# aleflabo/PREGO

Measured on AMD Instinct MI355X. Metric: frames/sec (per-frame action logits) on Assembly101-O TSN features, higher is better.
Workload: dtype fp16; 1 GPU; BASELINE configs[1]: Assembly101-O-test-split-shaped eval set, MiniROAD eval path (rgb+flow fp32 [T,2048] each -> per-frame probs[86] + argmax); clips_per_gpu=182, frames_per_gpu=2306143, min_T=3342, max_T=33981, flow=non-zero (full K=4096 layer1 GEMM), parallelism=clip-sharded dp1, no collective: every rank its own eval-set-sized clip list, weights=random init, seed 20

## Files before the change

prego_amd/csrc/ff_pass.hip:

```cpp
#include "common.h"
#include "kernels.h"
#include "gemm_tile.h"
#include "pass_handshake.h"

#define FF_TIMEOUT_TICKS 200000000ull

__device__ __forceinline__ bool ffp_wait_ge(const unsigned* p, unsigned need, unsigned* abort_word, unsigned code) {
  if (__hip_atomic_load(p, __ATOMIC_RELAXED, __HIP_MEMORY_SCOPE_AGENT) >= need) return true;
  const unsigned long long t0 = __builtin_amdgcn_s_memrealtime();
  unsigned spins = 0;
  for (;;) {
    __builtin_amdgcn_s_sleep(8);
    if (__hip_atomic_load(p, __ATOMIC_RELAXED, __HIP_MEMORY_SCOPE_AGENT) >= need) return true;
    if ((++spins & 31u) == 0u) {
      if (__hip_atomic_load(abort_word, __ATOMIC_RELAXED, __HIP_MEMORY_SCOPE_AGENT)) return false;
      if (__builtin_amdgcn_s_memrealtime() - t0 > FF_TIMEOUT_TICKS) {
        __hip_atomic_store(abort_word, code, __ATOMIC_RELAXED, __HIP_MEMORY_SCOPE_AGENT);
        return false;
      }
    }
  }
}

template <typename OT, bool SC1OUT>
// ... 23 lines not shown
#pragma unroll
  for (int y = 0; y < 2; ++y)
#pragma unroll
    for (int j = 0; j < 2; ++j) bv[y][j] = *(const float4*)(bias + y * 128 + wc * 32 + fq * 8 + j * 4);
  const __amdgpu_buffer_rsrc_t rs_c = __builtin_amdgcn_make_buffer_rsrc((void*)C, 0, rows * ldc * 2, 0x00020000);
#pragma unroll
  for (int x = 0; x < 2; ++x)
#pragma unroll
    for (int y = 0; y < 2; ++y) {
      const int n = y * 128 + wc * 32 + fq * 8;
#pragma unroll
      for (int i = 0; i < 4; ++i) {
        const int m = x * 128 + grp * 64 + i * 16 + fr;
        const f32x4 v0 = acc[x][y][i][0], v1 = acc[x][y][i][1];
        u32x4 pk;
        pk[0] = op16<OT>::pack2_sat(v0[0] + bv[y][0].x, v0[1] + bv[y][0].y); pk[1] = op16<OT>::pack2_sat(v0[2] + bv[y][0].z, v0[3] + bv[y][0].w);
        pk[2] = op16<OT>::pack2_sat(v1[0] + bv[y][1].x, v1[1] + bv[y][1].y); pk[3] = op16<OT>::pack2_sat(v1[2] + bv[y][1].z, v1[3] + bv[y][1].w);
        if constexpr (SC1OUT) __builtin_amdgcn_raw_buffer_store_b128(pk, rs_c, (m * ldc + n) * 2, 0, AUX_SC1);
        else __builtin_amdgcn_raw_buffer_store_b128(pk, rs_c, (m * ldc + n) * 2, 0, 0);
      }
    }
}

template <typename OT, bool IN16>
__device__ __forceinline__ void ffp_pack_rows(const FfPassArgs& a, int my_rows, int wave, int lane, const char* srgb, const char* sflow,
                                              bf16_t* __restrict__ Xs) {
  constexpr int ES = IN16 ? 2 : 4, NV = IN16 ? 1 : 2;
  constexpr int PR = 2;
  const int din = a.kx;
  const int cr_rgb = (a.d_rgb + 2047) >> 11, cpr = cr_rgb + ((a.d_flow + 2047) >> 11);
  const int n_rounds = my_rows > 0 ? ((my_rows + PR - 1) / PR) * cpr : 0;
  auto readlane_ptr = [](const char* p, int l) -> const char* {
    const unsigned long long v = (unsigned long long)p;
    const unsigned lo = (unsigned)__builtin_amdgcn_readlane((int)(unsigned)v, l), hi = (unsigned)__builtin_amdgcn_readlane((int)(unsigned)(v >> 32), l);
    return (const char*)(((unsigned long long)hi << 32) | lo);
  };
  int voff_in = lane * 8 * ES, voff_in2 = voff_in + 1024 * ES, voff_out = lane * 16;
  asm volatile("" : "+v"(voff_in), "+v"(voff_in2), "+v"(voff_out));
  auto issue = [&](u32x4 (&v)[PR][4][NV], int k) {
    const int rp = k / cpr, cj = k - rp * cpr;
    const bool fl = cj >= cr_rgb;
    const int cwin = (fl ? cj - cr_rgb : cj) << 11, seg_len = fl ? a.d_flow : a.d_rgb;
#pragma unroll
    for (int e = 0; e < PR; ++e) {
      const int r = rp * PR + e, rr = r < my_rows ? r : 0;
      const char* s0 = readlane_ptr(srgb, rr);
      const char* s1 = readlane_ptr(sflow, rr);
      const char* src = fl ? s1 : s0;
      const __amdgpu_buffer_rsrc_t rs = __builtin_amdgcn_make_buffer_rsrc((void*)(src + (size_t)cwin * ES), 0,
                                                                          (r < my_rows && src != nullptr) ? (seg_len - cwin) * ES : 0, 0x00020000);
#pragma unroll
      for (int b = 0; b < 4; ++b)
#pragma unroll
        for (int w = 0; w < NV; ++w)
          v[e][b][w] = __builtin_amdgcn_raw_buffer_load_b128(rs, (b < 2 ? voff_in : voff_in2) + ((b & 1) * 512 * ES + 16 * w), 0, AUX_NT);
    }
  };
  auto drain = [&](const u32x4 (&v)[PR][4][NV], int k) {
    const int rp = k / cpr, cj = k - rp * cpr;
    const bool fl = cj >= cr_rgb;
    const int cwin = (fl ? cj - cr_rgb : cj) << 11, seg_len = fl ? a.d_flow : a.d_rgb, seg_base = fl ? a.d_rgb : 0;
#pragma unroll
    for (int e = 0; e < PR; ++e) {
      const int r = rp * PR + e;
      bf16_t* dst = Xs + (size_t)(wave * 32 + (r < my_rows ? r : 0)) * din + seg_base + cwin;
      const __amdgpu_buffer_rsrc_t rs = __builtin_amdgcn_make_buffer_rsrc((void*)dst, 0, r < my_rows ? (seg_len - cwin) * 2 : 0, 0x00020000);
#pragma unroll
      for (int b = 0; b < 4; ++b) {
        u32x4 o = v[e][b][0];
        if constexpr (!IN16) {
          const u32x4 x = v[e][b][0], y = v[e][b][NV - 1];
          o[0] = op16<OT>::pack2_sat(__uint_as_float(x[0]), __uint_as_float(x[1])); o[1] = op16<OT>::pack2_sat(__uint_as_float(x[2]), __uint_as_float(x[3]));
          o[2] = op16<OT>::pack2_sat(__uint_as_float(y[0]), __uint_as_float(y[1])); o[3] = op16<OT>::pack2_sat(__uint_as_float(y[2]), __uint_as_float(y[3]));
        }
        __builtin_amdgcn_raw_buffer_store_b128(o, rs, voff_out + b * 1024, 0, 0);
      }
    }
  };
  u32x4 va[PR][4][NV], vb[PR][4][NV];
  if (n_rounds == 0) return;
  issue(va, 0);
  int k = 0;
#define PACK_FENCE() __builtin_amdgcn_sched_barrier(0)
  for (; k + 2 < n_rounds; k += 2) {
    issue(vb, k + 1); PACK_FENCE();
    drain(va, k); PACK_FENCE();
    issue(va, k + 2); PACK_FENCE();
    drain(vb, k + 1); PACK_FENCE();
  }
  if (k + 1 < n_rounds) {
    issue(vb, k + 1); PACK_FENCE();
    drain(va, k); PACK_FENCE();
    drain(vb, k + 1);
  } else {
    drain(va, k);
  }
#undef PACK_FENCE
}

template <typename OT>
__device__ __forceinline__ void ffp_pack(const FfPassArgs& a, int row0, int nrows, bf16_t* __restrict__ Xs) {
  int tid_ = threadIdx.x;
  asm volatile("" : "+v"(tid_));
  const int lane = tid_ & 63, wave = __builtin_amdgcn_readfirstlane(tid_ >> 6);
  const int rl = wave * 32 + (lane & 31);
  int clip = 0, t = 0;
  if (rl < nrows) {
    const int row = row0 + rl;
    int lo = a.plan.blk_step[row >> 5];
    while (lo + 1 < a.plan.s_max && a.plan.rowoff[lo + 1] <= row) ++lo;
    const int slot = row - a.plan.rowoff[lo];
    int k = a.plan.seg_off[slot];
    const int kend = a.plan.seg_off[slot + 1];
    while (k + 1 < kend && a.plan.seg_start[k + 1] <= lo) ++k;
    clip = a.plan.seg_clip[k];
    t = lo - a.plan.seg_start[k];
    if (a.rowmap != nullptr && lane < 32) ((int2*)a.rowmap)[row] = make_int2(clip, t);
  }
  const char* srgb = nullptr; const char* sflow = nullptr;
  const int es = a.in16 ? 2 : 4;
  if (rl < nrows) {
    const float* rgb = a.rgb_ptrs ? a.rgb_ptrs[clip] : nullptr;
    const float* flow = a.flow_ptrs ? a.flow_ptrs[clip] : nullptr;
    if (rgb) srgb = (const char*)rgb + (size_t)t * a.d_rgb * es;
    if (flow) sflow = (const char*)flow + (size_t)t * a.d_flow * es;
  }
  const int my_rows = nrows - wave * 32 < 32 ? nrows - wave * 32 : 32;
  if (a.in16) ffp_pack_rows<OT, true>(a, my_rows, wave, lane, srgb, sflow, Xs);
  else ffp_pack_rows<OT, false>(a, my_rows, wave, lane, srgb, sflow, Xs);
}

constexpr int FLN_MAX_E = 2048;

template <typename OT, int NV, int NR>
__device__ __forceinline__ void ffp_ln(const FfPassArgs& a, int nrows, const bf16_t* __restrict__ Ys, bf16_t* __restrict__ Es, const float* gb) {
  int tid_ = threadIdx.x;
  asm volatile("" : "+v"(tid_));
  const int lane = tid_ & 63, wave = __builtin_amdgcn_readfirstlane(tid_ >> 6);
  const int E = NV * 512;
  const float fE = (float)a.E;
  if (wave >= nrows) return;
  auto request = [&](u32x4 (&dst)[NR][NV], int rb) {
#pragma unroll
    for (int e = 0; e < NR; ++e) {
      int r = rb + 8 * e;
      if (r >= nrows) r = wave;
      const bf16_t* y = Ys + (size_t)r * E;
#pragma unroll
      for (int i = 0; i < NV; ++i) dst[e][i] = *(const u32x4*)(y + (i * 64 + lane) * 8);
    }
// ... 186 lines not shown
    default: ffp_ln_generic<OT, 8, 2>(a, nrows, Ys, Es); break;
  }
}

template <typename OT>
__global__ __launch_bounds__(512, 2) void ff_pass_kernel(FfPassArgs a) {
  extern __shared__ __attribute__((aligned(16))) char smem[];
  __shared__ int s_job[2];
  const int tid = threadIdx.x;
  const int xcc = __builtin_amdgcn_readfirstlane(__builtin_amdgcn_s_getreg((3 << 11) | 20) & 7);
  if (xcc < a.xcd_lo) return;
  if (tid == 0) {
    const unsigned nth = __hip_atomic_fetch_add(a.hs.ff_here + xcc, 1u, __ATOMIC_RELAXED, __HIP_MEMORY_SCOPE_AGENT);
    s_job[1] = hs_wait(a.hs, a.hs.ticks_all) == PREGO_HS_GO ? 1 : 0;
    if (a.max_wg > 0 && (int)nth >= a.max_wg) s_job[1] = 0;
  }
  __syncthreads();
  if (!__builtin_amdgcn_readfirstlane(s_job[1])) return;
  __shared__ __attribute__((aligned(16))) float s_gb[2 * FLN_MAX_E];
  if (a.E <= FLN_MAX_E)
    for (int c = tid; c < a.E; c += 512) { s_gb[c] = a.ln_g[c]; s_gb[FLN_MAX_E + c] = a.ln_b[c]; }
  const int q = xcc - a.xcd_lo, nf = 8 - a.xcd_lo;
  const int n_q = a.n_units > q ? (a.n_units - q + nf - 1) / nf : 0;
  const int sg = a.sg, tpr = sg * (2 + a.nt1 + a.nt2);
  const int n_rounds = (n_q + sg - 1) / sg + a.lag3;
  __shared__ unsigned long long s_stat[11];
  const bool stats = a.stats != nullptr && tid == 0;
  if (stats) {
    for (int e = 0; e < 8; ++e) s_stat[e] = 0;
    s_stat[9] = __builtin_amdgcn_s_memrealtime(); s_stat[8] = s_stat[9]; s_stat[10] = __builtin_amdgcn_s_memtime();
  }
#define FSTAT(i) do { if (stats) { const unsigned long long n_ = __builtin_amdgcn_s_memrealtime(); s_stat[i] += n_ - s_stat[8]; s_stat[8] = n_; } } while (0)
  for (;;) {
    __syncthreads();
    if (tid == 0) s_job[0] = (int)__hip_atomic_fetch_add(a.tick + q, 1u, __ATOMIC_RELAXED, __HIP_MEMORY_SCOPE_AGENT);
    __syncthreads();
    const int k = __builtin_amdgcn_readfirstlane(s_job[0]);
    const int round = k / tpr, j = k - round * tpr;
    FSTAT(5);
    if (round >= n_rounds) break;
    int type, i, nb = 0;
    if (j < sg) { type = 0; i = round * sg + j; }
    else if (j < sg + sg * a.nt1) { const int jj = j - sg; type = 1; nb = jj / sg; i = (round - a.lag1) * sg + (jj - nb * sg); }
    else if (j < 2 * sg + sg * a.nt1) { type = 2; i = (round - a.lag2) * sg + (j - sg - sg * a.nt1); }
    else { const int jj = j - 2 * sg - sg * a.nt1; type = 3; nb = jj / sg; i = (round - a.lag3) * sg + (jj - nb * sg); }
    if (i < 0 || i >= n_q) continue;
    const int u = q + i * nf;
    if (tid == 0) {
      bool ok = true;
      const int up = u - a.ring_units;
      if (type == 0) {
        if (up >= 0) ok = ffp_wait_ge(a.l1_cnt + up, (unsigned)a.nt1, a.abort_word, 0x100u);
      } else if (type == 1) {
        ok = ffp_wait_ge(a.pack_done + u, 1u, a.abort_word, 0x101u);
        if (ok && up >= 0) ok = ffp_wait_ge(a.ln_done + up, 1u, a.abort_word, 0x102u);
      } else if (type == 2) {
        ok = ffp_wait_ge(a.l1_cnt + u, (unsigned)a.nt1, a.abort_word, 0x103u);
        if (ok && up >= 0) ok = ffp_wait_ge(a.wih_cnt + up, (unsigned)a.nt2, a.abort_word, 0x104u);
      } else {
        ok = ffp_wait_ge(a.ln_done + u, 1u, a.abort_word, 0x105u);
        const int ug = u - a.gi_ring_units;
        if (ok && ug >= 0) ok = ffp_wait_ge(a.rec_cnt + (ug >> a.chunk_unit_shift), (unsigned)a.rec_expect, a.abort_word, 0x106u);
      }
      s_job[1] = ok ? 1 : 0;
    }
    __syncthreads();
    if (!__builtin_amdgcn_readfirstlane(s_job[1])) break;
    FSTAT(4);
    asm volatile("buffer_inv sc0" ::: "memory");
    const int row0 = u * 256;
    const int nrows = a.total_rows - row0 < 256 ? a.total_rows - row0 : 256;
    const size_t slot = (size_t)(u % a.ring_units) * 256;
    if (type == 0) {
      if (!(a.dbg & 1)) ffp_pack<OT>(a, row0, nrows, a.X + slot * a.kx);
    } else if (type == 1) {
      if (!(a.dbg & 4))
      ffp_tile<OT, false>(smem, a.X + slot * a.kx, a.kx, nrows, a.w1 + (size_t)nb * 256 * a.ld_w1, a.ld_w1, a.b1 + nb * 256,
                          a.Y + slot * a.E + nb * 256, a.E, a.kx);
    } else if (type == 2) {
      if (a.dbg & 2) { }
      else ffp_ln_any<OT>(a, nrows, a.Y + slot * a.E, a.Eb + slot * a.E, s_gb);
    } else {
      const size_t gslot = (size_t)(u & (a.gi_ring_units - 1)) * 256;
      if (!(a.dbg & 8))
      ffp_tile<OT, true>(smem, a.Eb + slot * a.E, a.E, nrows, a.w_ih + (size_t)nb * 256 * a.E, a.E, a.bias2 + nb * 256,
                         a.GI + gslot * a.n3 + nb * 256, a.n3, a.E);
    }
    asm volatile("s_waitcnt vmcnt(0)" ::: "memory");
    __syncthreads();
    FSTAT(type);
    if (tid == 0) {
      if (type == 0) __hip_atomic_store(a.pack_done + u, 1u, __ATOMIC_RELAXED, __HIP_MEMORY_SCOPE_AGENT);
      else if (type == 1) __hip_atomic_fetch_add(a.l1_cnt + u, 1u, __ATOMIC_RELAXED, __HIP_MEMORY_SCOPE_AGENT);
      else if (type == 2) __hip_atomic_store(a.ln_done + u, 1u, __ATOMIC_RELAXED, __HIP_MEMORY_SCOPE_AGENT);
      else {
        const unsigned old = __hip_atomic_fetch_add(a.wih_cnt + u, 1u, __ATOMIC_RELAXED, __HIP_MEMORY_SCOPE_AGENT);
        if (old + 1u == (unsigned)a.nt2)
          __hip_atomic_fetch_add(a.gi_cnt + (u >> a.chunk_unit_shift), 1u, __ATOMIC_RELAXED, __HIP_MEMORY_SCOPE_AGENT);
      }
    }
  }
  if (stats) {
    s_stat[7] = __builtin_amdgcn_s_memrealtime() - s_stat[9];
    s_stat[6] = __builtin_amdgcn_s_memtime() - s_stat[10];
    for (int e = 0; e < 8; ++e) atomicAdd(a.stats + e, s_stat[e]);
  }
#undef FSTAT
}

int launch_ff_pass(const FfPassArgs& a, hipStream_t s) {
  if (a.E % 512 || a.E > 4096 || a.kx % kPpBK || a.kx < 2 * kPpBK || a.n3 % 256 || a.xcd_lo < 1 || a.xcd_lo > 7) return -1;
  if (a.sg < 1 || a.ring_units % (8 - a.xcd_lo) || (a.gi_ring_units & (a.gi_ring_units - 1)) || a.nt1 != a.E / 256 || a.nt2 != a.n3 / 256) return -1;
  static DeviceOnce once;
  once.run([&] {
    (void)hipFuncSetAttribute((const void*)ff_pass_kernel<bf16_t>, hipFuncAttributeMaxDynamicSharedMemorySize, 2 * kPpBuf);
    (void)hipFuncSetAttribute((const void*)ff_pass_kernel<f16_t>, hipFuncAttributeMaxDynamicSharedMemorySize, 2 * kPpBuf);
  });
  if (a.f16) ff_pass_kernel<f16_t><<<256, 512, 2 * kPpBuf, s>>>(a);
  else ff_pass_kernel<bf16_t><<<256, 512, 2 * kPpBuf, s>>>(a);
  return 0;
}
```

prego_amd/csrc/head_softmax.hip:

```cpp
#include "common.h"
#include "kernels.h"
#include <cstdlib>

#define HM 4
template <typename WT, int NTC>
__global__ __launch_bounds__(256) void head_softmax_kernel(
    const WT* __restrict__ Hrelu,
    const WT* __restrict__ Wc,
    const float* __restrict__ bc,
    SlotPlan plan, int row0, int nrows, int HID, int C, int apply_softmax,
    float* const* __restrict__ out_ptrs,
    int* const* __restrict__ argmax_ptrs) {
  constexpr bool BF = (sizeof(WT) == 2);
  const int lane = threadIdx.x & 63, wave = threadIdx.x >> 6;
  const int l15 = lane & 15, l4 = lane >> 4;
  const int rbase = (blockIdx.x * 4 + wave) * 16 * HM;
  if (rbase >= nrows) return;
  int arow[HM];
#pragma unroll
  for (int m = 0; m < HM; ++m) { arow[m] = rbase + m * 16 + l15; if (arow[m] > nrows - 1) arow[m] = nrows - 1; }

  __shared__ unsigned long long s_out[4][64], s_arg[4][64];
  {
    typedef const __attribute__((address_space(4))) int* cint_p;
// ... 93 lines not shown
      for (int o = 1; o < 16; o <<= 1) s += __shfl_xor(s, o, 64);
      const float inv = 1.0f / s;
#pragma unroll
      for (int j = 0; j < NTC; ++j) v[j] *= inv;
    }
    const int rr = m * 16 + l4 * 4 + e;
    if (rbase + rr < nrows) {
      float* op = (float*)s_out[wave][rr];
      if (op) {
#pragma unroll
        for (int j = 0; j < NTC; ++j) {
          const int c = j * 16 + l15;
          if (c < C) op[c] = v[j];
        }
      }
      if (l15 == 0) {
        int* aptr = (int*)s_arg[wave][rr];
        if (aptr) *aptr = mi;
      }
    }
  }
}

template <int NTC, typename OT = bf16_t>
__global__ __launch_bounds__(256, 1) void head_softmax_v2_kernel(
    const bf16_t* __restrict__ Hrelu, const bf16_t* __restrict__ Wc, const float* __restrict__ bc, SlotPlan plan, int row0,
    int nrows, int C, int apply_softmax, float* const* __restrict__ out_ptrs, int* const* __restrict__ argmax_ptrs,
    const int2* __restrict__ rowmap ) {
  constexpr int HID = 1024, KS = 8;
  extern __shared__ __attribute__((aligned(16))) char smem[];
  f32x4* part = (f32x4*)smem;
  constexpr int PSTRIDE = 4 * 2 * NTC * 64;
  const int lane = threadIdx.x & 63, q = __builtin_amdgcn_readfirstlane(threadIdx.x >> 6);
  const int l15 = lane & 15, g = lane >> 4;
  bf16x8 wc[NTC][KS];
#pragma unroll
  for (int j = 0; j < NTC; ++j)
#pragma unroll
    for (int ks = 0; ks < KS; ++ks) wc[j][ks] = *(const bf16x8*)(Wc + (size_t)(j * 16 + l15) * HID + q * 256 + ks * 32 + 8 * g);
  float bias[NTC][4];
#pragma unroll
  for (int j = 0; j < NTC; ++j)
#pragma unroll
    for (int e = 0; e < 4; ++e) bias[j][e] = bc[j * 16 + 4 * g + e];

  const int nblk = (nrows + 31) / 32;
  const int* __restrict__ p_rowoff = plan.rowoff; const int* __restrict__ p_seg_off = plan.seg_off;
  const int* __restrict__ p_seg_clip = plan.seg_clip; const int* __restrict__ p_seg_start = plan.seg_start;
  const int* __restrict__ p_blk = plan.blk_step;
  const int s_max = plan.s_max;
  bf16x8 cur[2][KS], nxt[2][KS];
#define HEAD_LOAD(DST, BLK)                                                                                             \
  do {                                                                                                                  \
    _Pragma("unroll") for (int t = 0; t < 2; ++t) {                                                                     \
      int r_ = (BLK) * 32 + t * 16 + l15; if (r_ > nrows - 1) r_ = nrows - 1;                                           \
      _Pragma("unroll") for (int ks = 0; ks < KS; ++ks) {                                                               \
        const u32x4 v_ = __builtin_nontemporal_load((const u32x4*)(Hrelu + (size_t)r_ * HID + q * 256 + ks * 32 + 8 * g)); \
        DST[t][ks] = __builtin_bit_cast(bf16x8, v_);                                                                    \
      }                                                                                                                 \
    }                                                                                                                   \
  } while (0)
  const int rq = (q & 1) * 16 + l15;
  auto map_row = [&](int b) { int r = b * 32 + rq; return r < nrows ? r : nrows - 1; };
  int blk = blockIdx.x;
  int2 ct = make_int2(0, 0), ctn = make_int2(0, 0);
  if (blk < nblk) {
    if (rowmap != nullptr) ct = rowmap[map_row(blk)];
    HEAD_LOAD(cur, blk);
  }
  int parity = 0;
  for (; blk < nblk; blk += gridDim.x) {
    const int bn = blk + gridDim.x;
    const int bnc = bn < nblk ? bn : blk;
    float* op_raw = nullptr; int* ap_raw = nullptr;
    if (rowmap != nullptr) {
      op_raw = out_ptrs ? out_ptrs[ct.x] : nullptr;
      ap_raw = argmax_ptrs ? argmax_ptrs[ct.x] : nullptr;
      ctn = rowmap[map_row(bnc)];
    }
    __builtin_amdgcn_sched_barrier(0);
    HEAD_LOAD(nxt, bnc);
    __builtin_amdgcn_sched_barrier(0);
    float* op = nullptr; int* ap = nullptr;
    const int myrow = blk * 32 + q * 16 + l15;
    if (q < 2 && myrow < nrows && rowmap == nullptr) {
      const int row = row0 + myrow;
      int lo = p_blk[row >> 5];
      while (lo + 1 < s_max && p_rowoff[lo + 1] <= row) ++lo;
      const int slot = row - p_rowoff[lo];
      int k = p_seg_off[slot];
      const int kend = p_seg_off[slot + 1];
      while (k + 1 < kend && p_seg_start[k + 1] <= lo) ++k;
      const int clip = p_seg_clip[k], t = lo - p_seg_start[k];
      op = out_ptrs ? out_ptrs[clip] : nullptr;
      if (op) op += (size_t)t * C;
      ap = argmax_ptrs ? argmax_ptrs[clip] : nullptr;
      if (ap) ap += t;
    }
    f32x4 acc[2][NTC];
#pragma unroll
    for (int t = 0; t < 2; ++t)
#pragma unroll
      for (int j = 0; j < NTC; ++j) acc[t][j] = (f32x4){0.f, 0.f, 0.f, 0.f};
#pragma unroll
    for (int ks = 0; ks < KS; ++ks)
#pragma unroll
      for (int t = 0; t < 2; ++t)
#pragma unroll
        for (int j = 0; j < NTC; ++j) acc[t][j] = op16<OT>::mfma(wc[j][ks], cur[t][ks], acc[t][j]);
    f32x4* pw = part + parity * PSTRIDE;
    if (q != 0) {
#pragma unroll
      for (int j = 0; j < NTC; ++j) pw[((q * 2 + 0) * NTC + j) * 64 + lane] = acc[0][j];
    }
    if (q != 1) {
#pragma unroll
      for (int j = 0; j < NTC; ++j) pw[((q * 2 + 1) * NTC + j) * 64 + lane] = acc[1][j];
    }
    __syncthreads();
    if (q < 2 && myrow < nrows && rowmap != nullptr) {
      op = op_raw;
      if (op) op += (size_t)ct.y * C;
      ap = ap_raw;
      if (ap) ap += ct.y;
    }
    if (q < 2) {
      float v[NTC][4];
#pragma unroll
      for (int j = 0; j < NTC; ++j) {
        const f32x4 mine = q == 0 ? acc[0][j] : acc[1][j];
        f32x4 sum = (f32x4){0.f, 0.f, 0.f, 0.f};
#pragma unroll
        for (int src = 0; src < 4; ++src) {
          const f32x4 p = (src == q) ? mine : pw[((src * 2 + q) * NTC + j) * 64 + lane];
          sum[0] += p[0]; sum[1] += p[1]; sum[2] += p[2]; sum[3] += p[3];
        }
        v[j][0] = sum[0] + bias[j][0]; v[j][1] = sum[1] + bias[j][1]; v[j][2] = sum[2] + bias[j][2]; v[j][3] = sum[3] + bias[j][3];
      }
      float mx = -INFINITY; int mi = 0x7fffffff;
#pragma unroll
      for (int j = 0; j < NTC; ++j)
#pragma unroll
        for (int e = 0; e < 4; ++e) {
          const int c = j * 16 + 4 * g + e;
          if (c < C && v[j][e] > mx) { mx = v[j][e]; mi = c; }
        }
#pragma unroll
      for (int o = 16; o < 64; o <<= 1) {
        const float omx = __shfl_xor(mx, o, 64);
        const int omi = __shfl_xor(mi, o, 64);
        if (omx > mx || (omx == mx && omi < mi)) { mx = omx; mi = omi; }
      }
      if (apply_softmax) {
        float sm = 0.f;
#pragma unroll
        for (int j = 0; j < NTC; ++j)
#pragma unroll
          for (int e = 0; e < 4; ++e) {
            const int c = j * 16 + 4 * g + e;
            v[j][e] = c < C ? __expf(v[j][e] - mx) : 0.f;
            sm += v[j][e];
          }
        sm += __shfl_xor(sm, 16, 64);
        sm += __shfl_xor(sm, 32, 64);
        const float inv = 1.0f / sm;
#pragma unroll
        for (int j = 0; j < NTC; ++j)
#pragma unroll
          for (int e = 0; e < 4; ++e) v[j][e] *= inv;
      }
      if (op) {
#pragma unroll
        for (int j = 0; j < NTC; ++j) {
          const int c = j * 16 + 4 * g;
          if (c + 3 < C && ((C & 3) == 0)) *(float4*)(op + c) = make_float4(v[j][0], v[j][1], v[j][2], v[j][3]);
          else {
#pragma unroll
            for (int e = 0; e < 4; ++e) if (c + e < C) op[c + e] = v[j][e];
          }
        }
      }
      if (ap && g == 0) *ap = mi;
    }
    parity ^= 1;
    __builtin_amdgcn_sched_barrier(0);
#pragma unroll
    for (int t = 0; t < 2; ++t)
#pragma unroll
      for (int ks = 0; ks < KS; ++ks) cur[t][ks] = nxt[t][ks];
    ct = ctn;
  }
#undef HEAD_LOAD
}

int launch_head_softmax(bool bf16, const void* Hrelu, const void* Wc, const float* bc, const SlotPlan& plan,
                        int row0, int nrows, int hid, int C, int apply_softmax,
                        float* const* out_ptrs, int* const* argmax_ptrs, hipStream_t s, const void* rowmap, bool f16) {
  if (nrows <= 0) return 0;
  const int ntc = (C + 15) / 16;
  static const bool no_v2 = prego_tune_env("PREGO_HEAD_V1") != nullptr;
  if (bf16 && hid == 1024 && ntc <= 6 && !no_v2) {
    const int nblk = (nrows + 31) / 32;
    const int grid2 = nblk < 256 ? nblk : 256;
#define HV2(N)                                                                                                      \
  case N: {                                                                                                         \
    const size_t lds = (size_t)2 * 4 * 2 * N * 64 * 16;                                                             \
    static DeviceOnce once;                                                                                         \
    once.run([&] { (void)hipFuncSetAttribute((const void*)head_softmax_v2_kernel<N>, hipFuncAttributeMaxDynamicSharedMemorySize, (int)lds);   \
                   (void)hipFuncSetAttribute((const void*)head_softmax_v2_kernel<N, f16_t>, hipFuncAttributeMaxDynamicSharedMemorySize, (int)lds); }); \
    if (f16) head_softmax_v2_kernel<N, f16_t><<<grid2, 256, lds, s>>>((const bf16_t*)Hrelu, (const bf16_t*)Wc, bc, plan, row0, nrows, C,  \
                                                                     apply_softmax, out_ptrs, argmax_ptrs, (const int2*)rowmap);    \
    else head_softmax_v2_kernel<N><<<grid2, 256, lds, s>>>((const bf16_t*)Hrelu, (const bf16_t*)Wc, bc, plan, row0, nrows, C,  \
                                                      apply_softmax, out_ptrs, argmax_ptrs, (const int2*)rowmap);    \
    return 0;                                                                                                       \
  }
    switch (ntc) { HV2(1) HV2(2) HV2(3) HV2(4) HV2(5) HV2(6) default: break; }
#undef HV2
  }
  const int grid = (nrows + 64 * HM - 1) / (64 * HM);
#define HL(WT, N)                                                                                             \
  head_softmax_kernel<WT, N><<<grid, 256, 0, s>>>((const WT*)Hrelu, (const WT*)Wc, bc, plan, row0, nrows,     \
                                                  hid, C, apply_softmax, out_ptrs, argmax_ptrs)
#define HD(N)                          \
  case N:                              \
    if (bf16 && f16) HL(f16_t, N);     \
    else if (bf16) HL(bf16_t, N);      \
    else HL(float, N);                 \
    break
  switch (ntc) {
    HD(1); HD(2); HD(3); HD(4); HD(5); HD(6); HD(7); HD(8);
    default: return -1;
  }
#undef HD
#undef HL
  return 0;
}
```

prego_amd/csrc/kernels.h:

```cpp
#pragma once
#include <hip/hip_runtime_api.h>
#include <stddef.h>
#include <stdint.h>
#include <mutex>

const char* prego_tune_env(const char* name);

struct DeviceOnce {
  std::mutex mu;
  bool done[64] = {};
  template <class F> int run(F&& f) {
    int dev = 0;
    (void)hipGetDevice(&dev);
    if (dev < 0 || dev >= 64) { f(); return 0; }
    std::lock_guard<std::mutex> g(mu);
    if (!done[dev]) { f(); done[dev] = true; }
    return dev;
  }
};

#ifndef PREGO_HAVE_SLOTPLAN
struct SlotPlan {
  const int* rowoff; const int* nact; const int* seg_off; const int* seg_clip; const int* seg_start; const int* blk_step;
  int s_max; int n_slots;
// ... 40 lines not shown
  int no_mt;
  const unsigned* gi_cnt;
  unsigned* rec_cnt;
  int chunk_shift, n_chunks;
  int units_per_chunk, units_last;
  unsigned gi_row_mask;
  PassHandshake hs;
  float out_floor;
};
struct FfPassArgs {
  const float* const* rgb_ptrs; const float* const* flow_ptrs;
  SlotPlan plan;
  void* rowmap;
  int d_rgb, d_flow;
  int in16;
  int kx;
  const unsigned short* w1; int ld_w1; const float* b1;
  const float* ln_g; const float* ln_b; float ln_eps;
  const unsigned short* w_ih; const float* bias2;
  int E, n3;
  unsigned short* X; unsigned short* Y; unsigned short* Eb;
  unsigned short* GI;
  int ring_units, gi_ring_units;
  int total_rows, n_units;
  int xcd_lo;
  int chunk_unit_shift;
  int rec_expect;
  int nt1, nt2;
  int sg;
  int max_wg;
  int lag1, lag2, lag3;
  int dbg;
  unsigned long long* stats;
  int f16;
  unsigned* tick;
  unsigned* pack_done; unsigned* l1_cnt; unsigned* ln_done; unsigned* wih_cnt;
  unsigned* gi_cnt;
  const unsigned* rec_cnt;
  unsigned* abort_word;
  PassHandshake hs;
};
int launch_ff_pass(const FfPassArgs& a, hipStream_t s);
int launch_gru_recurrence_pass(int hid, GruArgs a, hipStream_t s);
int gru_group_size(bool bf16, int hid);
bool gru_hidden_supported(bool bf16, int hid);

// ... 406 lines not shown
```

prego_amd/csrc/miniroad_split.cpp:

```cpp
#include "miniroad_handle.h"

#include <algorithm>
#include <chrono>
#include <cstdlib>
#include <mutex>
#include <thread>

static int tuned_pow2(const char* name, int dflt) {
  const char* v = prego_tune_env(name);
  const int x = v ? atoi(v) : 0;
  return (x >= 16 && (x & (x - 1)) == 0) ? x : dflt;
}
static int split_gi_ring_units(int R) { return tuned_pow2("PREGO_SPLIT_GI_RING", R <= 3 ? 32 : 256); }
static const int kSplitRingPerXcd = (prego_tune_env("PREGO_SPLIT_RING_PER_XCD") && atoi(prego_tune_env("PREGO_SPLIT_RING_PER_XCD")) >= 12 &&
                                     atoi(prego_tune_env("PREGO_SPLIT_RING_PER_XCD")) % 4 == 0) ? atoi(prego_tune_env("PREGO_SPLIT_RING_PER_XCD")) : 24;
static const int kSplitSg = (prego_tune_env("PREGO_SPLIT_SG") && kSplitRingPerXcd % std::max(1, atoi(prego_tune_env("PREGO_SPLIT_SG"))) == 0)
                                ? std::max(1, atoi(prego_tune_env("PREGO_SPLIT_SG"))) : 2;
static int split_chunk_shift(int R) { return prego_tune_env("PREGO_SPLIT_CHUNK_SHIFT") ? atoi(prego_tune_env("PREGO_SPLIT_CHUNK_SHIFT")) : (R <= 3 ? 3 : 6); }
SplitRings split_rings(const prego_miniroad* h, int R) {
  SplitRings g;
  g.ring_units = kSplitRingPerXcd * (8 - R);
  g.x = align_up((size_t)g.ring_units * 256 * (size_t)(h->d_rgb + h->d_flow) * 2, 256);
  g.y = align_up((size_t)g.ring_units * 256 * (size_t)h->emb * 2, 256);
  g.e = g.y;
  g.gi = align_up((size_t)split_gi_ring_units(R) * 256 * (size_t)3 * h->hid * 2, 256);
  g.total = g.x + g.y + g.e + g.gi;
  return g;
}
bool split_workspace_ok(const prego_miniroad* h, int R, size_t workspace_bytes) { return workspace_bytes >= split_rings(h, R).total; }

size_t split_buf_need(const prego_miniroad* h, long long total) {
  const long long n_units = (total + 255) / 256;
  const int shift = split_chunk_shift(1);
  const long long n_chunks = (n_units + (1 << shift) - 1) >> shift;
  return align_up((size_t)total * h->hid * 2, 256) + align_up((size_t)total * 8, 256) + align_up(((size_t)4 * n_units + 2 * (size_t)n_chunks + 32) * 4, 256);
}
bool split_resident_ok(const prego_miniroad* h, long long total) { return h->res_buf && split_buf_need(h, total) <= h->res_bytes; }

extern "C" size_t prego_miniroad_resident_bytes(const prego_miniroad* h, int n_clips, const int32_t* lens, int flags) {
  if (!h || n_clips <= 0 || !lens) return 0;
  if ((flags & PREGO_FWD_KEEP) || h->layers != 1) return 0;
// ... 38 lines not shown
  HIPCHK(hipMemsetAsync(h->h_state, 0, (size_t)h->n_slots * H * 4, s));
  PassHandshake hs{};
  h->hs_seq = (h->hs_seq + 1u) & 0x3FFFFFFFu;
  if (h->hs_seq == 0u) h->hs_seq = 1u;
  hs.word = hs_word; hs.ff_here = ff_here; hs.host = h->pin_hs; hs.seq = h->hs_seq; hs.ticks_lead = 5000000u; hs.ticks_all = 10000000u;
  int fault = 0;
#ifdef PREGO_DEBUG_ABI
  fault = h->dbg_fault; h->dbg_fault = 0;
  if (fault == 3 || fault == 4) {
    HIPCHK(hipMemsetD32Async((hipDeviceptr_t)hs_word, PREGO_HS_GO, 1, s));
    HIPCHK(hipMemsetD32Async((hipDeviceptr_t)ff_here, 1, 8, s));
    if (fault == 3) HIPCHK(hipMemsetD32Async((hipDeviceptr_t)rec_cnt, R * h->P * 4, n_chunks, s));
    else HIPCHK(hipMemsetD32Async((hipDeviceptr_t)gi_cnt, upc, n_chunks, s));
    hs.host = nullptr;
  }
#endif

  FfPassArgs fa{};
  fa.rgb_ptrs = tb.rgb; fa.flow_ptrs = with_flow ? tb.flow : nullptr; fa.plan = plan; fa.rowmap = RM;
  fa.d_rgb = h->d_rgb; fa.d_flow = with_flow ? h->d_flow : 0; fa.in16 = in16 ? 1 : 0; fa.kx = kx;
  fa.w1 = (const unsigned short*)h->w1; fa.ld_w1 = din; fa.b1 = h->b1; fa.ln_g = h->ln_g; fa.ln_b = h->ln_b; fa.ln_eps = 1e-5f;
  fa.w_ih = (const unsigned short*)h->w_ih_perm; fa.bias2 = h->bias2_perm; fa.E = E; fa.n3 = 3 * H;
  fa.X = X; fa.Y = Y; fa.Eb = Eb; fa.GI = GI; fa.ring_units = rg.ring_units; fa.gi_ring_units = gi_ring;
  fa.total_rows = total; fa.n_units = n_units; fa.xcd_lo = R; fa.chunk_unit_shift = chunk_shift;
  fa.rec_expect = R * h->P * 4; fa.nt1 = E / 256; fa.nt2 = 3 * H / 256;
  static const int lag1 = prego_tune_env("PREGO_SPLIT_LAG1") ? atoi(prego_tune_env("PREGO_SPLIT_LAG1")) : 2;
  static const int lag2 = prego_tune_env("PREGO_SPLIT_LAG2") ? atoi(prego_tune_env("PREGO_SPLIT_LAG2")) : 3;
  static const int lag3 = prego_tune_env("PREGO_SPLIT_LAG3") ? atoi(prego_tune_env("PREGO_SPLIT_LAG3")) : 4;
  static const bool want_stats = prego_tune_env("PREGO_SPLIT_STATS") != nullptr;
  fa.sg = kSplitSg; fa.lag1 = lag1; fa.lag2 = lag2; fa.lag3 = lag3; fa.f16 = h->f16 ? 1 : 0;
  static const int ff_cus = prego_tune_env("PREGO_SPLIT_FF_CUS") ? atoi(prego_tune_env("PREGO_SPLIT_FF_CUS")) : 0;
  fa.max_wg = ff_cus;
  fa.stats = want_stats ? h->stamps : nullptr;
#ifdef PREGO_DEBUG_ABI
  static const int dbg = prego_tune_env("PREGO_SPLIT_DBG") ? atoi(prego_tune_env("PREGO_SPLIT_DBG")) : 0;
  fa.dbg = dbg;
#endif
  fa.tick = tick; fa.pack_done = pack_done; fa.l1_cnt = l1_cnt; fa.ln_done = ln_done; fa.wih_cnt = wih_cnt; fa.gi_cnt = gi_cnt;
  fa.rec_cnt = rec_cnt; fa.abort_word = h->abort_word; fa.hs = hs;
  const int ring_sr = kSplitRingPerXcd / kSplitSg;
  if (lag1 < 1 || lag2 <= lag1 || lag3 <= lag2 || lag1 >= ring_sr || lag2 - ring_sr >= lag1 || lag3 - ring_sr >= lag2)
    return prego_fail_(PREGO_EINVAL, "split pass: lags %d %d %d", lag1, lag2, lag3);

  GruArgs ga{};
  ga.whh = h->w_hh; ga.b_hn = h->b_hn; ga.gi = GI; ga.gi_bf16 = 1; ga.f16 = h->f16 ? 1 : 0; ga.h_relu_out = HR; ga.h_raw_out = nullptr;
  ga.h_state = h->h_state; ga.hx = h->hx; ga.flags = h->flags; ga.abort_word = h->abort_word;
  ga.rowoff = h->d_rowoff; ga.nact = h->d_nact; ga.t0 = 0; ga.t1 = h->t_max; ga.row_base = 0; ga.rows = 0;
  ga.n_clips = h->n_slots; ga.G = h->G; ga.seg_off = h->plan_single ? nullptr : h->d_seg_off;
  ga.seg_start = h->plan_single ? nullptr : h->d_seg_start; ga.stamps = (h->use_stamps && !want_stats) ? h->stamps : nullptr;
  ga.sync = h->flags; ga.armed = 0; ga.Gd = R;
  ga.gi_cnt = gi_cnt; ga.rec_cnt = rec_cnt; ga.chunk_shift = chunk_shift + 8; ga.n_chunks = n_chunks;
// ... 80 lines not shown
```

Before: 25.08 million frames/s.

## Split pack jobs into quarters, retune lags, double-buffer head softmax kernel

The feed-forward pass now splits each 256-row pack job into four 64-row sub-jobs with a counting pack_done, so layer-1 tiles can start as soon as all quarters finish and packing spreads across more workgroups. When R<=3 the pipeline lags are shortened by one. A separate gi_lead_units parameter gates GI ring reuse, but with the default of 0 it falls back to the ring size. The head softmax kernel is rewritten to ping-pong two row buffers without register copies, keep bias in shared memory, and specialize on whether rowmap is present. These changes carry more job-dispatch and atomic overhead, and the smaller lags raise the risk of waiting.

```diff
diff --git a/prego_amd/csrc/ff_pass.hip b/prego_amd/csrc/ff_pass.hip
--- a/prego_amd/csrc/ff_pass.hip
+++ b/prego_amd/csrc/ff_pass.hip
@@ -69,6 +69,10 @@
     }
 }
 
+constexpr int kPackQ = 4;
+constexpr int kPackRows = 256 / kPackQ;
+constexpr int kPackWaveRows = kPackRows / 8;
+
 template <typename OT, bool IN16>
 __device__ __forceinline__ void ffp_pack_rows(const FfPassArgs& a, int my_rows, int wave, int lane, const char* srgb, const char* sflow,
                                               bf16_t* __restrict__ Xs) {
@@ -110,7 +114,7 @@
 #pragma unroll
     for (int e = 0; e < PR; ++e) {
       const int r = rp * PR + e;
-      bf16_t* dst = Xs + (size_t)(wave * 32 + (r < my_rows ? r : 0)) * din + seg_base + cwin;
+      bf16_t* dst = Xs + (size_t)(wave * kPackWaveRows + (r < my_rows ? r : 0)) * din + seg_base + cwin;
       const __amdgpu_buffer_rsrc_t rs = __builtin_amdgcn_make_buffer_rsrc((void*)dst, 0, r < my_rows ? (seg_len - cwin) * 2 : 0, 0x00020000);
 #pragma unroll
       for (int b = 0; b < 4; ++b) {
@@ -150,7 +154,7 @@
   int tid_ = threadIdx.x;
   asm volatile("" : "+v"(tid_));
   const int lane = tid_ & 63, wave = __builtin_amdgcn_readfirstlane(tid_ >> 6);
-  const int rl = wave * 32 + (lane & 31);
+  const int rl = wave * kPackWaveRows + (lane & (kPackWaveRows - 1));
   int clip = 0, t = 0;
   if (rl < nrows) {
     const int row = row0 + rl;
@@ -162,7 +166,7 @@
     while (k + 1 < kend && a.plan.seg_start[k + 1] <= lo) ++k;
     clip = a.plan.seg_clip[k];
     t = lo - a.plan.seg_start[k];
-    if (a.rowmap != nullptr && lane < 32) ((int2*)a.rowmap)[row] = make_int2(clip, t);
+    if (a.rowmap != nullptr && lane < kPackWaveRows) ((int2*)a.rowmap)[row] = make_int2(clip, t);
   }
   const char* srgb = nullptr; const char* sflow = nullptr;
   const int es = a.in16 ? 2 : 4;
@@ -172,7 +176,7 @@
     if (rgb) srgb = (const char*)rgb + (size_t)t * a.d_rgb * es;
     if (flow) sflow = (const char*)flow + (size_t)t * a.d_flow * es;
   }
-  const int my_rows = nrows - wave * 32 < 32 ? nrows - wave * 32 : 32;
+  const int my_rows = nrows - wave * kPackWaveRows < kPackWaveRows ? nrows - wave * kPackWaveRows : kPackWaveRows;
   if (a.in16) ffp_pack_rows<OT, true>(a, my_rows, wave, lane, srgb, sflow, Xs);
   else ffp_pack_rows<OT, false>(a, my_rows, wave, lane, srgb, sflow, Xs);
 }
@@ -405,7 +409,7 @@
     for (int c = tid; c < a.E; c += 512) { s_gb[c] = a.ln_g[c]; s_gb[FLN_MAX_E + c] = a.ln_b[c]; }
   const int q = xcc - a.xcd_lo, nf = 8 - a.xcd_lo;
   const int n_q = a.n_units > q ? (a.n_units - q + nf - 1) / nf : 0;
-  const int sg = a.sg, tpr = sg * (2 + a.nt1 + a.nt2);
+  const int sg = a.sg, np = sg * kPackQ, tpr = np + sg * (1 + a.nt1 + a.nt2);
   const int n_rounds = (n_q + sg - 1) / sg + a.lag3;
   __shared__ unsigned long long s_stat[11];
   const bool stats = a.stats != nullptr && tid == 0;
@@ -423,10 +427,10 @@
     FSTAT(5);
     if (round >= n_rounds) break;
     int type, i, nb = 0;
-    if (j < sg) { type = 0; i = round * sg + j; }
-    else if (j < sg + sg * a.nt1) { const int jj = j - sg; type = 1; nb = jj / sg; i = (round - a.lag1) * sg + (jj - nb * sg); }
-    else if (j < 2 * sg + sg * a.nt1) { type = 2; i = (round - a.lag2) * sg + (j - sg - sg * a.nt1); }
-    else { const int jj = j - 2 * sg - sg * a.nt1; type = 3; nb = jj / sg; i = (round - a.lag3) * sg + (jj - nb * sg); }
+    if (j < np) { type = 0; nb = j % kPackQ; i = round * sg + j / kPackQ; }
+    else if (j < np + sg * a.nt1) { const int jj = j - np; type = 1; nb = jj / sg; i = (round - a.lag1) * sg + (jj - nb * sg); }
+    else if (j < np + sg + sg * a.nt1) { type = 2; i = (round - a.lag2) * sg + (j - np - sg * a.nt1); }
+    else { const int jj = j - np - sg - sg * a.nt1; type = 3; nb = jj / sg; i = (round - a.lag3) * sg + (jj - nb * sg); }
     if (i < 0 || i >= n_q) continue;
     const int u = q + i * nf;
     if (tid == 0) {
@@ -435,14 +439,14 @@
       if (type == 0) {
         if (up >= 0) ok = ffp_wait_ge(a.l1_cnt + up, (unsigned)a.nt1, a.abort_word, 0x100u);
       } else if (type == 1) {
-        ok = ffp_wait_ge(a.pack_done + u, 1u, a.abort_word, 0x101u);
+        ok = ffp_wait_ge(a.pack_done + u, (unsigned)kPackQ, a.abort_word, 0x101u);
         if (ok && up >= 0) ok = ffp_wait_ge(a.ln_done + up, 1u, a.abort_word, 0x102u);
       } else if (type == 2) {
         ok = ffp_wait_ge(a.l1_cnt + u, (unsigned)a.nt1, a.abort_word, 0x103u);
         if (ok && up >= 0) ok = ffp_wait_ge(a.wih_cnt + up, (unsigned)a.nt2, a.abort_word, 0x104u);
       } else {
         ok = ffp_wait_ge(a.ln_done + u, 1u, a.abort_word, 0x105u);
-        const int ug = u - a.gi_ring_units;
+        const int ug = u - a.gi_lead_units;
         if (ok && ug >= 0) ok = ffp_wait_ge(a.rec_cnt + (ug >> a.chunk_unit_shift), (unsigned)a.rec_expect, a.abort_word, 0x106u);
       }
       s_job[1] = ok ? 1 : 0;
@@ -455,7 +459,8 @@
     const int nrows = a.total_rows - row0 < 256 ? a.total_rows - row0 : 256;
     const size_t slot = (size_t)(u % a.ring_units) * 256;
     if (type == 0) {
-      if (!(a.dbg & 1)) ffp_pack<OT>(a, row0, nrows, a.X + slot * a.kx);
+      const int qrow = nb * kPackRows, qn = nrows - qrow < kPackRows ? nrows - qrow : kPackRows;
+      if (!(a.dbg & 1)) ffp_pack<OT>(a, row0 + qrow, qn, a.X + (slot + qrow) * a.kx);
     } else if (type == 1) {
       if (!(a.dbg & 4))
       ffp_tile<OT, false>(smem, a.X + slot * a.kx, a.kx, nrows, a.w1 + (size_t)nb * 256 * a.ld_w1, a.ld_w1, a.b1 + nb * 256,
@@ -473,7 +478,7 @@
     __syncthreads();
     FSTAT(type);
     if (tid == 0) {
-      if (type == 0) __hip_atomic_store(a.pack_done + u, 1u, __ATOMIC_RELAXED, __HIP_MEMORY_SCOPE_AGENT);
+      if (type == 0) __hip_atomic_fetch_add(a.pack_done + u, 1u, __ATOMIC_RELAXED, __HIP_MEMORY_SCOPE_AGENT);
       else if (type == 1) __hip_atomic_fetch_add(a.l1_cnt + u, 1u, __ATOMIC_RELAXED, __HIP_MEMORY_SCOPE_AGENT);
       else if (type == 2) __hip_atomic_store(a.ln_done + u, 1u, __ATOMIC_RELAXED, __HIP_MEMORY_SCOPE_AGENT);
       else {
@@ -493,7 +498,7 @@
 
 int launch_ff_pass(const FfPassArgs& a, hipStream_t s) {
   if (a.E % 512 || a.E > 4096 || a.kx % kPpBK || a.kx < 2 * kPpBK || a.n3 % 256 || a.xcd_lo < 1 || a.xcd_lo > 7) return -1;
-  if (a.sg < 1 || a.ring_units % (8 - a.xcd_lo) || (a.gi_ring_units & (a.gi_ring_units - 1)) || a.nt1 != a.E / 256 || a.nt2 != a.n3 / 256) return -1;
+  if (a.sg < 1 || a.ring_units % (8 - a.xcd_lo) || (a.gi_ring_units & (a.gi_ring_units - 1)) || a.gi_lead_units < 1 || a.gi_lead_units > a.gi_ring_units || a.nt1 != a.E / 256 || a.nt2 != a.n3 / 256) return -1;
   static DeviceOnce once;
   once.run([&] {
     (void)hipFuncSetAttribute((const void*)ff_pass_kernel<bf16_t>, hipFuncAttributeMaxDynamicSharedMemorySize, 2 * kPpBuf);
diff --git a/prego_amd/csrc/head_softmax.hip b/prego_amd/csrc/head_softmax.hip
--- a/prego_amd/csrc/head_softmax.hip
+++ b/prego_amd/csrc/head_softmax.hip
@@ -139,7 +139,7 @@
   }
 }
 
-template <int NTC, typename OT = bf16_t>
+template <int NTC, typename OT, bool MAP >
 __global__ __launch_bounds__(256, 1) void head_softmax_v2_kernel(
     const bf16_t* __restrict__ Hrelu, const bf16_t* __restrict__ Wc, const float* __restrict__ bc, SlotPlan plan, int row0,
     int nrows, int C, int apply_softmax, float* const* __restrict__ out_ptrs, int* const* __restrict__ argmax_ptrs,
@@ -155,19 +155,16 @@
   for (int j = 0; j < NTC; ++j)
 #pragma unroll
     for (int ks = 0; ks < KS; ++ks) wc[j][ks] = *(const bf16x8*)(Wc + (size_t)(j * 16 + l15) * HID + q * 256 + ks * 32 + 8 * g);
-  float bias[NTC][4];
-#pragma unroll
-  for (int j = 0; j < NTC; ++j)
-#pragma unroll
-    for (int e = 0; e < 4; ++e) bias[j][e] = bc[j * 16 + 4 * g + e];
+  __shared__ __attribute__((aligned(16))) float s_bias[16 * NTC];
+  if (threadIdx.x < 16 * NTC) s_bias[threadIdx.x] = bc[threadIdx.x];
 
   const int nblk = (nrows + 31) / 32;
   const int* __restrict__ p_rowoff = plan.rowoff; const int* __restrict__ p_seg_off = plan.seg_off;
   const int* __restrict__ p_seg_clip = plan.seg_clip; const int* __restrict__ p_seg_start = plan.seg_start;
   const int* __restrict__ p_blk = plan.blk_step;
   const int s_max = plan.s_max;
-  bf16x8 cur[2][KS], nxt[2][KS];
-#define HEAD_LOAD(DST, BLK)                                                                                             \
+  bf16x8 rows[2][2][KS];
+#define HEAD_LOAD(DST, BLK)                                                                                           \
   do {                                                                                                                  \
     _Pragma("unroll") for (int t = 0; t < 2; ++t) {                                                                     \
       int r_ = (BLK) * 32 + t * 16 + l15; if (r_ > nrows - 1) r_ = nrows - 1;                                           \
@@ -179,28 +176,30 @@
   } while (0)
   const int rq = (q & 1) * 16 + l15;
   auto map_row = [&](int b) { int r = b * 32 + rq; return r < nrows ? r : nrows - 1; };
+  const int gstep = gridDim.x;
   int blk = blockIdx.x;
-  int2 ct = make_int2(0, 0), ctn = make_int2(0, 0);
-  if (blk < nblk) {
-    if (rowmap != nullptr) ct = rowmap[map_row(blk)];
-    HEAD_LOAD(cur, blk);
-  }
+  if (blk >= nblk) return;
+  auto exists = [&](int b) { return b < nblk ? b : (int)blockIdx.x; };
+  int2 ct[2] = {make_int2(0, 0), make_int2(0, 0)};
+  float* op_raw[2] = {nullptr, nullptr}; int* ap_raw[2] = {nullptr, nullptr};
+  float* const* const otab = out_ptrs ? out_ptrs : (float* const*)argmax_ptrs;
+  int* const* const atab = argmax_ptrs ? argmax_ptrs : (int* const*)out_ptrs;
+  if constexpr (MAP) {
+    ct[0] = rowmap[map_row(blk)];
+    op_raw[0] = otab[ct[0].x];
+    ap_raw[0] = atab[ct[0].x];
+  }
+  __builtin_amdgcn_sched_barrier(0);
+  HEAD_LOAD(rows[0], blk);
+  __builtin_amdgcn_sched_barrier(0);
+  if constexpr (MAP) ct[1] = rowmap[map_row(exists(blk + gstep))];
+  HEAD_LOAD(rows[1], exists(blk + gstep));
+  __builtin_amdgcn_sched_barrier(0);
   int parity = 0;
-  for (; blk < nblk; blk += gridDim.x) {
-    const int bn = blk + gridDim.x;
-    const int bnc = bn < nblk ? bn : blk;
-    float* op_raw = nullptr; int* ap_raw = nullptr;
-    if (rowmap != nullptr) {
-      op_raw = out_ptrs ? out_ptrs[ct.x] : nullptr;
-      ap_raw = argmax_ptrs ? argmax_ptrs[ct.x] : nullptr;
-      ctn = rowmap[map_row(bnc)];
-    }
-    __builtin_amdgcn_sched_barrier(0);
-    HEAD_LOAD(nxt, bnc);
-    __builtin_amdgcn_sched_barrier(0);
+  auto head_block = [&](const bf16x8 (&cur)[2][KS], const int b, const int2 ct_s, float* op_s, int* ap_s) __attribute__((always_inline)) {
     float* op = nullptr; int* ap = nullptr;
-    const int myrow = blk * 32 + q * 16 + l15;
-    if (q < 2 && myrow < nrows && rowmap == nullptr) {
+    const int myrow = b * 32 + q * 16 + l15;
+    if (!MAP && q < 2 && myrow < nrows) {
       const int row = row0 + myrow;
       int lo = p_blk[row >> 5];
       while (lo + 1 < s_max && p_rowoff[lo + 1] <= row) ++lo;
@@ -226,33 +225,30 @@
 #pragma unroll
         for (int j = 0; j < NTC; ++j) acc[t][j] = op16<OT>::mfma(wc[j][ks], cur[t][ks], acc[t][j]);
     f32x4* pw = part + parity * PSTRIDE;
-    if (q != 0) {
-#pragma unroll
-      for (int j = 0; j < NTC; ++j) pw[((q * 2 + 0) * NTC + j) * 64 + lane] = acc[0][j];
-    }
-    if (q != 1) {
-#pragma unroll
-      for (int j = 0; j < NTC; ++j) pw[((q * 2 + 1) * NTC + j) * 64 + lane] = acc[1][j];
-    }
+#pragma unroll
+    for (int t = 0; t < 2; ++t)
+#pragma unroll
+      for (int j = 0; j < NTC; ++j) pw[((q * 2 + t) * NTC + j) * 64 + lane] = acc[t][j];
     __syncthreads();
-    if (q < 2 && myrow < nrows && rowmap != nullptr) {
-      op = op_raw;
-      if (op) op += (size_t)ct.y * C;
-      ap = ap_raw;
-      if (ap) ap += ct.y;
+    if (MAP && q < 2 && myrow < nrows) {
+      op = out_ptrs ? op_s : nullptr;
+      if (op) op += (size_t)ct_s.y * C;
+      ap = argmax_ptrs ? ap_s : nullptr;
+      if (ap) ap += ct_s.y;
     }
     if (q < 2) {
       float v[NTC][4];
 #pragma unroll
       for (int j = 0; j < NTC; ++j) {
-        const f32x4 mine = q == 0 ? acc[0][j] : acc[1][j];
         f32x4 sum = (f32x4){0.f, 0.f, 0.f, 0.f};
 #pragma unroll
         for (int src = 0; src < 4; ++src) {
-          const f32x4 p = (src == q) ? mine : pw[((src * 2 + q) * NTC + j) * 64 + lane];
+          const f32x4 p = pw[((src * 2 + q) * NTC + j) * 64 + lane];
           sum[0] += p[0]; sum[1] += p[1]; sum[2] += p[2]; sum[3] += p[3];
         }
-        v[j][0] = sum[0] + bias[j][0]; v[j][1] = sum[1] + bias[j][1]; v[j][2] = sum[2] + bias[j][2]; v[j][3] = sum[3] + bias[j][3];
+        const float4 bj = *(const float4*)(s_bias + j * 16 + 4 * g);
+        v[j][0] = sum[0] + bj.x; v[j][1] = sum[1] + bj.y; v[j][2] = sum[2] + bj.z; v[j][3] = sum[3] + bj.w;
+        if (j & 1) __builtin_amdgcn_sched_barrier(0);
       }
       float mx = -INFINITY; int mi = 0x7fffffff;
 #pragma unroll
@@ -286,26 +282,41 @@
 #pragma unroll
           for (int e = 0; e < 4; ++e) v[j][e] *= inv;
       }
+      typedef __attribute__((address_space(1))) float gfloat_t;
+      typedef __attribute__((address_space(1))) int gint_t;
+      typedef __attribute__((address_space(1))) f32x4 gfloat4_t;
       if (op) {
+        gfloat_t* const og = (gfloat_t*)op;
 #pragma unroll
         for (int j = 0; j < NTC; ++j) {
           const int c = j * 16 + 4 * g;
-          if (c + 3 < C && ((C & 3) == 0)) *(float4*)(op + c) = make_float4(v[j][0], v[j][1], v[j][2], v[j][3]);
+          if (c + 3 < C && ((C & 3) == 0)) *(gfloat4_t*)(og + c) = (f32x4){v[j][0], v[j][1], v[j][2], v[j][3]};
           else {
 #pragma unroll
-            for (int e = 0; e < 4; ++e) if (c + e < C) op[c + e] = v[j][e];
+            for (int e = 0; e < 4; ++e) if (c + e < C) og[c + e] = v[j][e];
           }
         }
       }
-      if (ap && g == 0) *ap = mi;
+      if (ap && g == 0) *(gint_t*)ap = mi;
     }
     parity ^= 1;
+  };
+  auto head_request = [&](bf16x8 (&cur)[2][KS], int b2, int2& ct_s, const int2 ct_n, float*& op_n, int*& ap_n) __attribute__((always_inline)) {
     __builtin_amdgcn_sched_barrier(0);
-#pragma unroll
-    for (int t = 0; t < 2; ++t)
-#pragma unroll
-      for (int ks = 0; ks < KS; ++ks) cur[t][ks] = nxt[t][ks];
-    ct = ctn;
+    b2 = exists(b2);
+    if constexpr (MAP) {
+      op_n = otab[ct_n.x];
+      ap_n = atab[ct_n.x];
+      ct_s = rowmap[map_row(b2)];
+    }
+    HEAD_LOAD(cur, b2);
+    __builtin_amdgcn_sched_barrier(0);
+  };
+  for (; blk < nblk; blk += 2 * gstep) {
+    head_block(rows[0], blk, ct[0], op_raw[0], ap_raw[0]);
+    head_request(rows[0], blk + 2 * gstep, ct[0], ct[1], op_raw[1], ap_raw[1]);
+    head_block(rows[1], blk + gstep < nblk ? blk + gstep : nblk, ct[1], op_raw[1], ap_raw[1]);
+    head_request(rows[1], blk + 3 * gstep, ct[1], ct[0], op_raw[0], ap_raw[0]);
   }
 #undef HEAD_LOAD
 }
@@ -319,20 +330,24 @@
   if (bf16 && hid == 1024 && ntc <= 6 && !no_v2) {
     const int nblk = (nrows + 31) / 32;
     const int grid2 = nblk < 256 ? nblk : 256;
+    if (!out_ptrs && !argmax_ptrs) return 0;
+#define HV2K(N, T, M)                                                                                               \
+  head_softmax_v2_kernel<N, T, M><<<grid2, 256, lds, s>>>((const bf16_t*)Hrelu, (const bf16_t*)Wc, bc, plan, row0, nrows, C, apply_softmax, \
+                                                          out_ptrs, argmax_ptrs, (const int2*)rowmap)
+#define HV2A(N, T, M) (void)hipFuncSetAttribute((const void*)head_softmax_v2_kernel<N, T, M>, hipFuncAttributeMaxDynamicSharedMemorySize, (int)lds)
 #define HV2(N)                                                                                                      \
   case N: {                                                                                                         \
     const size_t lds = (size_t)2 * 4 * 2 * N * 64 * 16;                                                             \
     static DeviceOnce once;                                                                                         \
-    once.run([&] { (void)hipFuncSetAttribute((const void*)head_softmax_v2_kernel<N>, hipFuncAttributeMaxDynamicSharedMemorySize, (int)lds);   \
-                   (void)hipFuncSetAttribute((const void*)head_softmax_v2_kernel<N, f16_t>, hipFuncAttributeMaxDynamicSharedMemorySize, (int)lds); }); \
-    if (f16) head_softmax_v2_kernel<N, f16_t><<<grid2, 256, lds, s>>>((const bf16_t*)Hrelu, (const bf16_t*)Wc, bc, plan, row0, nrows, C,  \
-                                                                     apply_softmax, out_ptrs, argmax_ptrs, (const int2*)rowmap);    \
-    else head_softmax_v2_kernel<N><<<grid2, 256, lds, s>>>((const bf16_t*)Hrelu, (const bf16_t*)Wc, bc, plan, row0, nrows, C,  \
-                                                      apply_softmax, out_ptrs, argmax_ptrs, (const int2*)rowmap);    \
+    once.run([&] { HV2A(N, bf16_t, false); HV2A(N, bf16_t, true); HV2A(N, f16_t, false); HV2A(N, f16_t, true); });  \
+    if (f16) { if (rowmap) HV2K(N, f16_t, true); else HV2K(N, f16_t, false); }                                      \
+    else { if (rowmap) HV2K(N, bf16_t, true); else HV2K(N, bf16_t, false); }                                        \
     return 0;                                                                                                       \
   }
     switch (ntc) { HV2(1) HV2(2) HV2(3) HV2(4) HV2(5) HV2(6) default: break; }
 #undef HV2
+#undef HV2A
+#undef HV2K
   }
   const int grid = (nrows + 64 * HM - 1) / (64 * HM);
 #define HL(WT, N)                                                                                             \
diff --git a/prego_amd/csrc/kernels.h b/prego_amd/csrc/kernels.h
--- a/prego_amd/csrc/kernels.h
+++ b/prego_amd/csrc/kernels.h
@@ -86,6 +86,7 @@
   unsigned short* X; unsigned short* Y; unsigned short* Eb;
   unsigned short* GI;
   int ring_units, gi_ring_units;
+  int gi_lead_units;
   int total_rows, n_units;
   int xcd_lo;
   int chunk_unit_shift;
diff --git a/prego_amd/csrc/miniroad_split.cpp b/prego_amd/csrc/miniroad_split.cpp
--- a/prego_amd/csrc/miniroad_split.cpp
+++ b/prego_amd/csrc/miniroad_split.cpp
@@ -17,6 +17,12 @@
 static const int kSplitSg = (prego_tune_env("PREGO_SPLIT_SG") && kSplitRingPerXcd % std::max(1, atoi(prego_tune_env("PREGO_SPLIT_SG"))) == 0)
                                 ? std::max(1, atoi(prego_tune_env("PREGO_SPLIT_SG"))) : 2;
 static int split_chunk_shift(int R) { return prego_tune_env("PREGO_SPLIT_CHUNK_SHIFT") ? atoi(prego_tune_env("PREGO_SPLIT_CHUNK_SHIFT")) : (R <= 3 ? 3 : 6); }
+static const int kSplitGiLeadR3 = 0;
+static int split_gi_lead_units(int R, int ring, int upc) {
+  const char* v = prego_tune_env("PREGO_SPLIT_GI_LEAD");
+  const int x = v ? atoi(v) : (R <= 3 ? kSplitGiLeadR3 : 0);
+  return (x >= 2 * upc && x >= upc + (kSplitSg - 1) * (8 - R) && x <= ring && x % upc == 0) ? x : ring;
+}
 SplitRings split_rings(const prego_miniroad* h, int R) {
   SplitRings g;
   g.ring_units = kSplitRingPerXcd * (8 - R);
@@ -101,11 +107,14 @@
   fa.w1 = (const unsigned short*)h->w1; fa.ld_w1 = din; fa.b1 = h->b1; fa.ln_g = h->ln_g; fa.ln_b = h->ln_b; fa.ln_eps = 1e-5f;
   fa.w_ih = (const unsigned short*)h->w_ih_perm; fa.bias2 = h->bias2_perm; fa.E = E; fa.n3 = 3 * H;
   fa.X = X; fa.Y = Y; fa.Eb = Eb; fa.GI = GI; fa.ring_units = rg.ring_units; fa.gi_ring_units = gi_ring;
+  fa.gi_lead_units = split_gi_lead_units(R, gi_ring, upc);
   fa.total_rows = total; fa.n_units = n_units; fa.xcd_lo = R; fa.chunk_unit_shift = chunk_shift;
   fa.rec_expect = R * h->P * 4; fa.nt1 = E / 256; fa.nt2 = 3 * H / 256;
-  static const int lag1 = prego_tune_env("PREGO_SPLIT_LAG1") ? atoi(prego_tune_env("PREGO_SPLIT_LAG1")) : 2;
-  static const int lag2 = prego_tune_env("PREGO_SPLIT_LAG2") ? atoi(prego_tune_env("PREGO_SPLIT_LAG2")) : 3;
-  static const int lag3 = prego_tune_env("PREGO_SPLIT_LAG3") ? atoi(prego_tune_env("PREGO_SPLIT_LAG3")) : 4;
+  const int near_ = R <= 3 ? 1 : 0;
+  static const int lag1_env = prego_tune_env("PREGO_SPLIT_LAG1") ? atoi(prego_tune_env("PREGO_SPLIT_LAG1")) : 0;
+  static const int lag2_env = prego_tune_env("PREGO_SPLIT_LAG2") ? atoi(prego_tune_env("PREGO_SPLIT_LAG2")) : 0;
+  static const int lag3_env = prego_tune_env("PREGO_SPLIT_LAG3") ? atoi(prego_tune_env("PREGO_SPLIT_LAG3")) : 0;
+  const int lag1 = lag1_env ? lag1_env : 2 - near_, lag2 = lag2_env ? lag2_env : 3 - near_, lag3 = lag3_env ? lag3_env : 4 - near_;
   static const bool want_stats = prego_tune_env("PREGO_SPLIT_STATS") != nullptr;
   fa.sg = kSplitSg; fa.lag1 = lag1; fa.lag2 = lag2; fa.lag3 = lag3; fa.f16 = h->f16 ? 1 : 0;
   static const int ff_cus = prego_tune_env("PREGO_SPLIT_FF_CUS") ? atoi(prego_tune_env("PREGO_SPLIT_FF_CUS")) : 0;
```

Result: no change. 25.12 million frames/s, median of 4 (+0.2%).
